# dubhater/vapoursynth-mvtools

Measured on AMD Instinct MI355X. Metric: MDegrain3 cfg3 fps (Super+Analyse+Degrain end-to-end), higher is better.
Workload: dtype u16; 1 GPU; 4K YUV420P16 Degrain3 blksize=16 overlap=8 pel=2; batches_in_flight=2

## Files before the change

vapoursynth-mvtools_amd/csrc/mvx_analyse_spec.h:

```cpp
#pragma once
#include <type_traits>
#include "mvx_analyse_fast.h"

#define SPEC_TB 32
#define SPEC_STRIDE (SPEC_TB * 8 + 8)
#define SPEC_SLOTS_HEX 19
#define SPEC_SLOTS_EXH 29
#define MVX_FAST_NOSTRIP 8
#define MVX_FAST_NOSPEC 4

#ifdef MVX_SPEC_NOPACK
#define MVX_SPEC_PACK 0
#else
#define MVX_SPEC_PACK 1
#endif
#ifndef MVX_SPEC_PLANEORDER
#define MVX_SPEC_PLANEORDER 1
#endif
constexpr int SPEC_SW3 = 12;
#ifdef MVX_SPEC_PROF
#define SPROF_N 20
static __device__ unsigned long long g_specprof[SPROF_N];
#define SPROF(i) do { const long long t1_ = (long long)__builtin_amdgcn_s_memtime(); asm volatile("s_waitcnt lgkmcnt(0)" : : "s"(t1_) : "memory"); sprof[i] += t1_ - sprofT; sprofT = t1_; } while (0)
#else
#define SPROF(i) ((void)0)
#endif
#ifdef MVX_SPEC_PROF
#define SPEC_PROF_DUMP_() do { if (l == 0 && chain == 5 && S.role == 1) for (int i = 0; i < SPROF_N; i++) g_specprof[i] = (unsigned long long)S.sprof[i]; } while (0)
#else
#define SPEC_PROF_DUMP_() ((void)0)
#endif
#ifdef MVX_SPEC_STATS
static __device__ unsigned long long g_specstat[MVX_MAX_LEVELS][10];
#endif

template <int BPS, int BW, bool UV, int SWIN = 12, bool TEAM = false, bool SIDE = false> struct SpecSearcher : FastSearcher<BPS, BW, UV, 48> {
    typedef FastSearcher<BPS, BW, UV, 48> F;
    typedef FGeo<BPS, BW> G;
    using F::P; using F::J; using F::lds; using F::ldsRow; using F::ldsHist; using F::histBins;
    using F::nBlkX; using F::nBlkY; using F::pel; using F::logPel; using F::pw; using F::ph; using F::hpad; using F::vpad;
    using F::srcY; using F::srcU; using F::srcV; using F::refY; using F::refU; using F::refV; using F::srcUV; using F::refUV;
    using F::pitchY; using F::pitchC; using F::pstrideY; using F::pstrideC; using F::shadowY; using F::vectors;
    using F::chroma; using F::searchType; using F::nSearchParam; using F::penaltyNew; using F::penaltyZero; using F::pglobal; using F::badrange; using F::badcount; using F::fieldShift;
    using F::badSAD; using F::LSAD; using F::gmvx; using F::gmvy;
    using F::x0; using F::y0; using F::blkIdx; using F::nDxMin; using F::nDyMin; using F::nDxMax; using F::nDyMax;
    using F::predX; using F::predY; using F::pX; using F::pY; using F::nLambda; using F::bestX; using F::bestY; using F::bestSad;
    int ldsTab;
    int role, nw;
    lds_u8 *shRow;
    LDS_AS int *ctl;
    __device__ __forceinline__ int team_advance(int g, int c0, int lo, int hiE, bool fwd, int stepX, int hps) const {
        auto clampAt = [&](int v, int li) { const int xb = stepX * (c0 + li); return min(max(v, -((xb + hps) << logPel)), ((pw - xb - hpad - BW - hpad + hps) << logPel) - 1); };
        if (clampAt(g, lo) == g && clampAt(g, hiE - 1) == g) return g;
        for (int i = 0; i < hiE - lo; i++) g = clampAt(g, fwd ? lo + i : hiE - 1 - i);
        return g;
    }
    __device__ __forceinline__ void team_wait_ge(int need) const {
#ifdef MVX_TEAM_WATCHDOG
        unsigned spins = 0;
#endif
        while (uni(__hip_atomic_load(ctl, __ATOMIC_ACQUIRE, __HIP_MEMORY_SCOPE_WORKGROUP)) < need) {
            __builtin_amdgcn_s_sleep(2);
#ifdef MVX_TEAM_WATCHDOG
            if (++spins > (1u << 26)) __builtin_trap();
#endif
        }
    }
    __device__ __forceinline__ void team_acquire(int myG, int &px, int &py, int &ps) {
        team_wait_ge(myG);
        px = uni(__hip_atomic_load(ctl + 1, __ATOMIC_RELAXED, __HIP_MEMORY_SCOPE_WORKGROUP));
        py = uni(__hip_atomic_load(ctl + 2, __ATOMIC_RELAXED, __HIP_MEMORY_SCOPE_WORKGROUP));
        ps = uni(__hip_atomic_load(ctl + 3, __ATOMIC_RELAXED, __HIP_MEMORY_SCOPE_WORKGROUP));
        badcount = uni(__hip_atomic_load(ctl + 4, __ATOMIC_RELAXED, __HIP_MEMORY_SCOPE_WORKGROUP));
    }
    __device__ __forceinline__ void team_release(int done, int px, int py, int ps) const {
        if (lane_id() == 0) {
            __hip_atomic_store(ctl + 1, px, __ATOMIC_RELAXED, __HIP_MEMORY_SCOPE_WORKGROUP);
            __hip_atomic_store(ctl + 2, py, __ATOMIC_RELAXED, __HIP_MEMORY_SCOPE_WORKGROUP);
            __hip_atomic_store(ctl + 3, ps, __ATOMIC_RELAXED, __HIP_MEMORY_SCOPE_WORKGROUP);
            __hip_atomic_store(ctl + 4, badcount, __ATOMIC_RELAXED, __HIP_MEMORY_SCOPE_WORKGROUP);
        }
        __builtin_amdgcn_fence(__ATOMIC_RELEASE, "workgroup");
        if (lane_id() == 0) __hip_atomic_store(ctl, done, __ATOMIC_RELEASE, __HIP_MEMORY_SCOPE_WORKGROUP);
    }
#ifdef MVX_SPEC_PROF
    long long sprof[SPROF_N], sprofT;
// ... 38 lines not shown
        oA = luma_off_at(bx0, vx, vy) + (unsigned)rowA * pitchY + (unsigned)xbA;
        oB = 2 * chroma_off_at(bx0, vx, vyc) + (unsigned)rowB * 2 * pitchC + (unsigned)xbB;
    }
    template <int LOGG, int WMAX> __device__ __forceinline__ v4u pass_issue(Pass<LOGG, WMAX> &T, int piece) const {
        typedef PG<LOGG, WMAX> Q;
        v4u v;
        if (piece < Q::NA) { v = F::template ld_ref<G::LCB>(refY + T.curA); T.curA += (unsigned)(Q::GG >> G::LLOGC) * pitchY; asm volatile("" : "+v"(T.curA) : : "memory"); }
        else { v = F::template ld_ref<G::UVCB>(refUV + T.curB); T.curB += (unsigned)(Q::GG >> G::UVLOGC) * 2 * pitchC; asm volatile("" : "+v"(T.curB) : : "memory"); }
        return v;
    }
    template <int LOGG, int WMAX> __device__ __forceinline__ void pass_prime(Pass<LOGG, WMAX> &T, unsigned oA, unsigned oB) const {
        typedef PG<LOGG, WMAX> Q;
        T.curA = oA; T.curB = oB;
#pragma unroll
        for (int k = 0; k < Q::W; k++) T.r[k] = pass_issue(T, k);
    }
    template <int LOGG, int WMAX, bool REFILL = true> __device__ __forceinline__ void pass_run(Pass<LOGG, WMAX> &T, int s, unsigned nA, unsigned nB) const {
        typedef PG<LOGG, WMAX> Q;
        const int rowA = s >> G::LLOGC, xbA = (s & (Q::CA - 1)) * G::LCB, rowB = s >> G::UVLOGC, xbB = (s & (Q::CB - 1)) * G::UVCB;
        const lds_u8 *spA = lds + rowA * G::LROWB + xbA, *spB = lds + G::UOFF + rowB * G::UVROWB + xbB;
        constexpr int lstepA = (Q::GG >> G::LLOGC) * G::LROWB, lstepB = (Q::GG >> G::UVLOGC) * G::UVROWB;
        auto src_piece = [&](int k) { return k < Q::NA ? F::template lds_piece<G::LCB>(spA + k * lstepA) : F::template lds_piece<G::UVCB>(spB + (k - Q::NA) * lstepB); };
        constexpr int D = MVX_SRC_AHEAD < Q::NT ? MVX_SRC_AHEAD : Q::NT;
        v4u a[D];
#pragma unroll
        for (int k = 0; k < D; k++) a[k] = src_piece(k);
        unsigned aL = 0, aC = 0;
#pragma unroll
        for (int k = 0; k < Q::NT; k++) {
            const v4u cur = a[k % D];
            if (k + D < Q::NT) a[k % D] = src_piece(k + D);
            if (k < Q::NA) aL = F::template sad_regs<G::LCB>(cur, T.r[k % Q::W], aL);
            else aC = F::template sad_regs<G::UVCB>(cur, T.r[k % Q::W], aC);
            asm volatile("" : "+v"(aL), "+v"(aC) : : "memory");
            const int kk = k + Q::W;
            if (kk == Q::NT) { T.curA = nA; T.curB = nB; }
            if (REFILL || kk < Q::NT) T.r[k % Q::W] = pass_issue(T, kk % Q::NT);
        }
        T.aL = aL; T.aC = aC;
    }

#ifndef MVX_STRIP32
#define MVX_STRIP32 0
#endif
    static constexpr bool STRIP_OK = (BPS == 2 && (BW == 16 || (MVX_STRIP32 && BW == 32))) || (BPS == 1 && BW == 16);
    static constexpr int COLB = BPS == 2 ? 16 : 8, ROWB = 8 * COLB;
    static constexpr int HC = STRIP_OK ? BW / 16 : 1, SW_BLOCKS = 8 / HC - 1, LPB = 2 * HC, LPC = SW_BLOCKS * LPB;
    static constexpr int pickSW(int nt, int w) { return w <= 1 ? 1 : (w <= nt && nt % w == 0) ? w : pickSW(nt, w - 1); }
    static constexpr int SNA = BW, SNB = UV ? BW / 2 : 0, SNT = SNA + SNB, SW = pickSW(SNT, (BW == 32 && SWIN > 12) ? 12 : SWIN), S_UV = SNA * ROWB, SSTG = SNT / 8;
    static constexpr bool SDMA = STRIP_OK && COLB == 16 && HC == 1 && SW == 24 && SNT == 24;
    static_assert(!SDMA || (SW == SNT && SSTG == 3), "SDMA: strip_run<true> issues exactly SW loads per pass, a strip is three loads per lane");
    static_assert(SW <= 63, "the wait for a strip is s_waitcnt vmcnt(SW)");
    static constexpr bool PACK = SDMA && MVX_SPEC_PACK;
    __device__ __forceinline__ static int hex_ord(int i) {
        if constexpr (MVX_SPEC_PLANEORDER != 0) return (int)(0xDCBA7630985421ull >> (4 * i)) & 15;
        else return i;
    }
    struct StripPass { v4u r[SW]; unsigned curA, curB, aL, aC; };
    __device__ __forceinline__ v4u strip_issue(StripPass &T, int piece) const {
        v4u v;
        if (piece < SNA) { v = F::template ld_ref<COLB>(refY + T.curA); T.curA += pitchY; asm volatile("" : "+v"(T.curA) : : "memory"); }
        else { v = F::template ld_ref<COLB>(refUV + T.curB); T.curB += 2 * pitchC; asm volatile("" : "+v"(T.curB) : : "memory"); }
        return v;
    }
    __device__ __forceinline__ void strip_prime(StripPass &T, unsigned oA, unsigned oB) const {
        T.curA = oA; T.curB = oB;
#pragma unroll
        for (int k = 0; k < SW; k++) T.r[k] = strip_issue(T, k);
    }
    template <bool REFILL> __device__ __forceinline__ void strip_run(StripPass &T, int p, unsigned nA, unsigned nB, int bufOff = 0) const {
        const lds_u8 *sp = lds + bufOff + p * COLB;
        auto src_piece = [&](int k) { return F::template lds_piece<COLB>(sp + (k < SNA ? k * ROWB : S_UV + (k - SNA) * ROWB)); };
        constexpr int D = MVX_SRC_AHEAD;
        v4u a[D];
#pragma unroll
        for (int k = 0; k < D; k++) a[k] = src_piece(k);
        unsigned aL = 0, aC = 0;
#pragma unroll
        for (int k = 0; k < SNT; k++) {
            const v4u cur = a[k % D];
            if (k + D < SNT) a[k % D] = src_piece(k + D);
            if (k < SNA) aL = F::template sad_regs<COLB>(cur, T.r[k % SW], aL);
            else aC = F::template sad_regs<COLB>(cur, T.r[k % SW], aC);
            asm volatile("" : "+v"(aL), "+v"(aC) : : "memory");
            const int kk = k + SW;
            if (kk == SNT) { T.curA = nA; T.curB = nB; }
            if (REFILL || kk < SNT) T.r[k % SW] = strip_issue(T, kk % SNT);
        }
        T.aL = aL; T.aC = aC;
    }
    static constexpr bool STRIP8_OK = UV && BPS == 1 && BW == 8;
    static constexpr int W8_BLOCKS = 15, R8A = 8, R8B = 4, R8T = R8A + R8B;
    static_assert(!SIDE || (STRIP_OK && HC == 1) || STRIP8_OK, "blocks side by side: the 16x16 and the 8-bit 8x8 row passes only");
    static constexpr int WBLK = STRIP_OK ? (SIDE ? 4 : SW_BLOCKS) : STRIP8_OK ? (SIDE ? 8 : W8_BLOCKS) : SPEC_TB;
    static constexpr int GT = SPEC_TB / WBLK * WBLK, FR = 2 * GT;
    static_assert(GT >= 1 && GT <= SPEC_TB && FR <= 64, "a group fits the table, a frame the wave");
    struct Strip8 { v4u r[R8T]; unsigned curA, curB; unsigned aL[4], aC[4]; };
    __device__ __forceinline__ v4u strip8_issue(Strip8 &T, int piece) const {
        v4u v;
        if (piece < R8A) { v = F::template ld_ref<16>(refY + T.curA); T.curA += pitchY; asm volatile("" : "+v"(T.curA) : : "memory"); }
        else { v = F::template ld_ref<16>(refUV + T.curB); T.curB += 2 * pitchC; asm volatile("" : "+v"(T.curB) : : "memory"); }
        return v;
    }
    __device__ __forceinline__ void strip8_prime(Strip8 &T, unsigned oA, unsigned oB) const {
        T.curA = oA; T.curB = oB;
#pragma unroll
// ... 65 lines not shown
        __builtin_amdgcn_s_barrier();

        if (smallestPlane) { searchType = P.nLevels == 1 ? P.searchType : P.searchTypeCoarse; nSearchParam = P.nLevels == 1 ? P.nPelSearch : P.nSearchParam; }
        else { searchType = lvl == 0 ? P.searchType : P.searchTypeCoarse; nSearchParam = lvl == 0 ? P.nPelSearch : P.nSearchParam; }
        searchType = uni(searchType); nSearchParam = uni(nSearchParam);
        fieldShift = uni(lvl == 0 ? J.fieldShift : 0);
        badSAD = uni(P.badSAD); badrange = uni(P.badrange); badcount = 0;
        gmvx = pel * globalX; gmvy = pel * globalY + fieldShift;
        int nLambdaLevel = P.lambda / (pel * pel);
        const int nScale = 1 << lvl;
        if (P.plevel == 1) nLambdaLevel = nLambdaLevel * nScale;
        else if (P.plevel == 2) nLambdaLevel = nLambdaLevel * nScale * nScale;
        nLambdaLevel = uni(nLambdaLevel);
        penaltyZero = uni(P.pzero); pglobal = uni(P.global ? P.pglobal : P.pzero); penaltyNew = uni(P.pnew); LSAD = uni((long long)P.lsad);
        const int stepX = uni(P.blkX - P.ovX), stepY = uni(P.blkY - P.ovY);
        const int hps = hpad >> lvl, vps = vpad >> lvl;
        const bool meander = uni(P.meander) != 0;
        LDS_AS v2u *rowbuf = (LDS_AS v2u *)(TEAM ? shRow : lds + ldsRow);
        lds_u8 *tab = TEAM ? lds + ldsTab : lds + ldsRow + ((nBlkX * 8 + 15) & ~15);
        this->pf_setup();
        SPROF(8);
        auto lambda_of = [&](int predSad) {
            const double scale = (double)LSAD / (double)(LSAD + (long long)(predSad >> 1));
            return (int)(long long)((double)(long long)nLambdaLevel * scale * scale);
        };
        const bool hexLevel = searchType == SearchHex2;
        const bool specLevel = specEnabled && !smallestPlane;
        int rdx = 0, rdy = 0;
        if (hexLevel) {
            const int g = l >> 2;
            if (g < 6) { rdx = tab8(HEX2X >> 8, g & 7); rdy = tab8(HEX2Y >> 8, g & 7); }
            else if (g < 14) { rdx = tab8(PACK8(0, 0, -1, 1, -1, -1, 1, 1), g - 6); rdy = tab8(PACK8(-1, 1, 0, 0, -1, 1, -1, 1), g - 6); }
        } else {
            const int g = l >> 1, k = g < 8 ? g : g - 8;
            if (g < 8) { rdx = tab8(PACK8(0, 0, -1, 1, -1, -1, 1, 1), k); rdy = tab8(PACK8(-1, 1, 0, 0, -1, 1, -1, 1), k); }
            else if (g < 16) { rdx = tab8(PACK8(-1, -1, 0, 0, 1, 1, -2, 2), k); rdy = tab8(PACK8(-2, 2, -2, 2, -2, 2, -1, -1), k); }
            else if (g < 24) { rdx = tab8(PACK8(-2, 2, -2, 2, -2, -2, 2, 2), k - 8); rdy = tab8(PACK8(0, 0, 1, 1, -2, 2, -2, 2), k - 8); }
        }
        unsigned sPat = 0, bPat0 = 0, bPat1 = 0;
        {
            constexpr bool side8 = STRIP8_OK && SIDE;
            constexpr bool side16 = SIDE;
            const int gb = side8 ? l >> 3 : STRIP8_OK ? (l >= 45 ? 3 : l >= 30 ? 2 : l >= 15 ? 1 : 0) : side16 ? min(l >> 3, 3) : min(l / LPC, 3);
            for (int q = 0; q < 8; q++) {
                int dx, dy;
                const int sIdx = STRIP8_OK ? q * 16 + (l >> 2) : (PACK && hexLevel && q >= 1) ? 8 + (8 * (q - 1) + (l >> 3)) % 6 : q * 8 + (l >> 3);
                if (q < 4) { pat_delta(hexLevel, (STRIP_OK && hexLevel) ? hex_ord(min(sIdx, 13)) : sIdx, dx, dy); sPat |= (unsigned)((dx & 15) | ((dy & 15) << 4)) << (8 * q); }
                pat_delta(hexLevel, q * (side8 ? 8 : 4) + gb, dx, dy);
                const unsigned b = (unsigned)((dx & 15) | ((dy & 15) << 4)) << (8 * (q & 3));
                if (q < 4) bPat0 |= b; else bPat1 |= b;
            }
        }
#ifdef MVX_SPEC_STATS
        unsigned long long st0 = 0, st1 = 0, st2 = 0, st3 = 0, st4 = 0, st5 = 0, st6 = 0, st7 = 0, st8 = 0, st9 = 0;
#endif

        int prevX = 0, prevY = 0, prevSad = 0;
        const int syncGroups = syncEvery > 0 ? max(1, (syncEvery + GT / 2) / GT) : 0;
        int syncCount = syncGroups - 1;
        int Gc = 0;
        const int nGrpRow = (nBlkX + GT - 1) / GT;
        for (int blky = 0; blky < nBlkY; blky++) {
            const bool fwd = (blky & 1) == 0 || !meander;
            const int dir = fwd ? 1 : -1;
            y0 = vpad + stepY * blky;
            nDyMax = (ph - y0 - BW - vpad + vps) << logPel;
            nDyMin = -((y0 - vpad + vps) << logPel);
            if constexpr (TEAM) gmvy = this->clipy(gmvy);
            const bool specRow = specLevel && blky > 0;
            const int ngrp = (nBlkX + FR - 1) / FR;
            for (int gi = 0; gi < ngrp; gi++) {
                const int grp = fwd ? gi : ngrp - 1 - gi;
                const int c0 = grp * FR, c = c0 + l;
                const int ncol = min(FR, nBlkX - c0);
                const bool in = l < ncol;
                v4u bOut = {0, 0, 0, 0};
                for (int hi = 0; hi < 2; hi++) {
                    const int h = fwd ? hi : 1 - hi;
                    const int lo = h * GT, hiE = min(lo + GT, ncol);
                    if (lo >= ncol) continue;
                    const int myG = Gc++;
                    bool teamHeld = false;
                    if constexpr (TEAM) {
                        if (uni(myG % nw) != role) {
                            gmvx = team_advance(gmvx, c0, lo, hiE, fwd, stepX, hps);
                            continue;
                        }
                        if (specRow) {
                            const int j = 2 * grp + h;
                            const bool fwdPrev = ((blky - 1) & 1) == 0 || !meander;
                            auto idxPrev = [&](int jj) { return fwdPrev ? jj : nGrpRow - 1 - jj; };
                            int need = (blky - 1) * nGrpRow + idxPrev(j) + 1;
                            if (blky == nBlkY - 1) { const int j2 = j + dir; if (j2 >= 0 && j2 < nGrpRow) need = max(need, (blky - 1) * nGrpRow + idxPrev(j2) + 1); }
                            SPROF(7);
                            team_wait_ge(need);
                            SPROF(16);
                        }
                    }
                    SPROF(7);
                    if (syncGroups && ++syncCount == syncGroups) { __builtin_amdgcn_s_barrier(); syncCount = 0; }
                    SPROF(0);
                    const bool act = l >= lo && l < hiE;
                    unsigned long long okmask = 0, flagmask = 0;
                    int rX = 0, rY = 0, rSad = 0;
                    int pkU = 0, pkAh = 0, pkH = 0, pkG = 0;
                    int lam = 0;
                    bool staged2G = false;
// ... 74 lines not shown
                                    }
                                }
#pragma unroll
                                for (int k = 0; k < 8; k++) {
                                    const int vx = wx + tab8(PACK8(0, 0, -1, 1, -1, -1, 1, 1), k), vy = wy + tab8(PACK8(-1, 1, 0, 0, -1, 1, -1, 1), k);
                                    const v2u t = tt[6 + k];
                                    const int cc = cnew(vx, vy, t);
                                    if (vok(vx, vy) && cc < best) { best = cc; bx = vx; by = vy; bs = tot(t); }
                                }
                            } else {
#pragma unroll 1
                                for (int k0 = 0; k0 < 24; k0 += 8) {
                                    v2u tt[8];
#pragma unroll
                                    for (int k = 0; k < 8; k++) tt[k] = rd(k0 + k);
#pragma unroll
                                    for (int k = 0; k < 8; k++) {
                                        int dx, dy;
                                        if (k0 == 0) { dx = tab8(PACK8(0, 0, -1, 1, -1, -1, 1, 1), k); dy = tab8(PACK8(-1, 1, 0, 0, -1, 1, -1, 1), k); }
                                        else if (k0 == 8) { dx = tab8(PACK8(-1, -1, 0, 0, 1, 1, -2, 2), k); dy = tab8(PACK8(-2, 2, -2, 2, -2, 2, -1, -1), k); }
                                        else { dx = tab8(PACK8(-2, 2, -2, 2, -2, -2, 2, 2), k); dy = tab8(PACK8(0, 0, 1, 1, -2, 2, -2, 2), k); }
                                        const int vx = wx + dx, vy = wy + dy;
                                        const v2u t = tt[k];
                                        const int cc = cnew(vx, vy, t);
                                        if (vok(vx, vy) && cc < best) { best = cc; bx = vx; by = vy; bs = tot(t); }
                                    }
                                }
                            }
                            return won;
                        };
                        bool staged2 = false;
                        int pBest = 0, pX_ = 0, pY_ = fieldShift, pSad = 0;

                        const int nb = hiE - lo;
                        const bool lumaStrips = STRIP_OK && !UV && !chroma && stripEnabled && stepX == (SIDE ? BW : BW / 2);
                        const bool streamed = (chroma && (hexLevel ? STREAM_HEX : STREAM_EXH)) || lumaStrips;
                        if (streamed) {
                            const int pkZ = pk(0, fieldShift);
                            const int slotUp = hexLevel ? 14 : 24, slotZ = hexLevel ? 16 : 26;
                            unsigned long long pbMask = __ballot(act), p3Mask = 0;

                            SPROF(1);
                            if constexpr (STRIP_OK) {
                                constexpr bool side = SIDE;
                                if (stripEnabled && stepX == (side ? BW : BW / 2) && (UV ? chroma != 0 : chroma == 0)) {
                                    constexpr int TC = side ? 2 : HC, SWB = side ? 4 : SW_BLOCKS, LPCr = SWB * LPB;
                                    static_assert(SWB == WBLK, "the group length is counted in these windows");
                                    const int nw = (nb + SWB - 1) / SWB;
                                    const int npat = hexLevel ? 14 : 24;
                                    pbMask = 0;
                                    staged2 = true;
                                    unsigned stripW = 0;
                                    unsigned packS = 0;
                                    int pkW = 0;
                                    int lq = l;
                                    asm volatile("" : "+v"(lq));
                                    int gS, pS, gB, rB, mB, hB;
                                    bool tail, idleB;
                                    auto roles = [&]() {
                                        lq = l;
                                        asm volatile("" : "+v"(lq));
                                        gS = lq >> 3; pS = lq & 7;
                                        gB = side ? min(lq >> 3, 3) : min(lq / LPC, 3);
                                        rB = side ? (lq & 7) : lq >= 4 * LPC ? (lq - 4 * LPC) % LPC : lq - LPC * gB; mB = rB / LPB; hB = rB % LPB;
                                        tail = lq >= 56; idleB = lq >= 4 * LPCr;
                                    };
                                    roles();
                                    constexpr int SBUF = SNT * ROWB;
                                    auto widx = [&](int i) { return fwd ? i : nw - 1 - i; };
                                    auto w_cand = [&](int st, int w, int q, int rj, int &slot, int &colW, bool &stripLane, int &srcOff, unsigned &oA, unsigned &oB) {
                                        const int f = lo + SWB * w, L = min(SWB, hiE - f);
                                        const int bxf = hpad + stepX * (c0 + f);
                                        const int bufW = SDMA ? (widx(w) & 1) * SBUF : 0;
                                        const bool stripWin = st == 2 && ((stripW >> w) & 1);
                                        const int meB = min(mB, L - 1), colB = f + meB;
                                        int bU = 0, bAh = 0, bG = 0, bH = 0, bW = 0;
                                        if (st == 1) {
                                            bU = __builtin_amdgcn_ds_bpermute(colB << 2, pkU); bAh = __builtin_amdgcn_ds_bpermute(colB << 2, pkAh);
                                            bG = __builtin_amdgcn_ds_bpermute(colB << 2, pkG); bH = __builtin_amdgcn_ds_bpermute(colB << 2, pkH);
                                        } else if (!stripWin) bW = __builtin_amdgcn_ds_bpermute(colB << 2, pkW);
                                        if (stripWin || (st == 1 && tail)) {
                                            const int p = st == 1 ? pS : pS, g = gS;
                                            int vx, vy, vyc;
                                            int fV = f, LV = L, bxV = bxf, bufV = bufW;
                                            if (st == 1) { vx = 0; vy = fieldShift; vyc = 0; slot = slotZ; }
                                            else {
                                                int sW = __builtin_amdgcn_readlane(pkW, f);
                                                int idx = q * 8 + g, sh = 8 * q;
                                                if constexpr (PACK) {
                                                    if (rj >= 0) {
                                                        const int w2 = widx(widx(w) + 1), f2 = lo + SWB * w2, L2 = min(SWB, hiE - f2);
                                                        const int sW2 = __builtin_amdgcn_readlane(pkW, f2);
                                                        const bool hi = g >= 6 - 2 * rj;
                                                        fV = hi ? f2 : f; LV = hi ? L2 : L; bxV = hpad + stepX * (c0 + fV); sW = hi ? sW2 : sW; bufV = hi ? SBUF - bufW : bufW;
                                                        idx = 8 + 2 * rj + g - (hi ? 6 : 0); sh = 8 * (1 + rj);
                                                    }
                                                }
                                                const int dd = (int)(sPat >> sh), dx = (dd << 28) >> 28, dy = (dd << 24) >> 28;
                                                vx = upx(sW) + dx; vy = upy(sW) + dy; vyc = vy;
                                                slot = idx < npat ? (hexLevel ? hex_ord(idx) : idx) : -1;
                                            }
                                            const int pe = min(p, TC * (LV - 1) + 2 * HC - 1) * COLB;
                                            if ((p % TC != 0) | (p / TC >= LV)) slot = -1;
                                            colW = fV + p / TC; stripLane = true; srcOff = bufV + p * COLB;
                                            oA = luma_off_at(bxV, vx, vy) + (unsigned)pe;
                                            oB = 2 * chroma_off_at(bxV, vx, vyc) + (unsigned)pe;
                                        } else {
                                            const int me = meB, col = colB;
                                            int base, dx = 0, dy = 0;
                                            if (st == 1) {
                                                base = gB == 0 ? bU : gB == 1 ? bAh : gB == 2 ? bG : bH;
                                                slot = gB == 0 ? slotUp : gB == 1 ? slotUp + 1 : slotZ + gB - 1;
                                            } else {
                                                base = bW;
                                                const int ci = q * 4 + gB;
                                                const int dd = (int)((q < 4 ? bPat0 : bPat1) >> (8 * (q & 3)));
                                                dx = (dd << 28) >> 28; dy = (dd << 24) >> 28;
                                                slot = ci < npat ? ci : -1;
                                            }
                                            const int bx0 = hpad + stepX * (c0 + col);
                                            const int xMax = (pw - bx0 - BW - hpad + hps) << logPel, xMin = -((bx0 - hpad + hps) << logPel);
                                            const int cxv = upx(base), cyv = upy(base), tx = cxv + dx, ty = cyv + dy;
                                            const bool ok = (tx >= xMin) & (ty >= nDyMin) & (tx < xMax) & (ty < nDyMax);
                                            const int vx = ok ? tx : cxv, vy = ok ? ty : cyv;
                                            if ((hB != 0) | (mB >= L) | idleB) slot = -1;
                                            colW = f + me; stripLane = false; srcOff = bufW + (TC * me + hB) * COLB;
                                            oA = luma_off_at(bx0, vx, vy) + (unsigned)(hB * COLB);
                                            oB = 2 * chroma_off_at(bx0, vx, vy) + (unsigned)(hB * COLB);
                                        }
                                    };
                                    A4x32 stg[SDMA ? 1 : SSTG];
                                    auto stage_issue = [&](int w, int buf) {
                                        const int f = lo + SWB * w, L = min(SWB, hiE - f), bx0 = hpad + stepX * (c0 + f), pe = min(pS, TC * (L - 1) + 2 * HC - 1) * COLB;
                                        if constexpr (SDMA) asm volatile("s_waitcnt lgkmcnt(0)" : : : "memory");
#pragma unroll
                                        for (int k = 0; k < SSTG; k++) {
                                            const int row = gS + 8 * k;
                                            gl_u8 *g = 8 * k < SNA ? srcY + (unsigned)(y0 + row) * pitchY + (unsigned)bx0 * BPS + (unsigned)pe
                                                                   : srcUV + (unsigned)((y0 >> 1) + row - SNA) * 2 * pitchC + (unsigned)(bx0 >> 1) * 2 * BPS + (unsigned)pe;
                                            if constexpr (SDMA) {
                                                const unsigned m0v = (unsigned)(unsigned long long)(lds + buf * SBUF + 8 * k * ROWB);
                                                asm volatile("s_mov_b32 m0, %1\n\tglobal_load_lds_dwordx4 %0, off" : : "v"(g), "s"(m0v) : "memory", "m0");
                                            } else stg[k] = ld_chunk_g(g, COLB);
                                        }
                                    };
                                    auto stage_store = [&]() {
                                        if constexpr (SDMA) asm volatile("s_waitcnt vmcnt(%0)" : : "n"(SW) : "memory");
                                        else {
#pragma unroll
                                            for (int k = 0; k < SSTG; k++) st_chunk_l(lds + (gS + 8 * k) * ROWB + pS * COLB, stg[k], COLB);
                                        }
                                    };
                                    auto npass = [&](int st, int w) { return st == 1 ? 1 : ((stripW >> w) & 1) ? (npat + 7) / 8 : (npat + 3) / 4; };
                                    auto run_stage = [&](int st, int wFrom, int wTo) {
                                        int wi = wFrom, w = widx(wFrom), q = 0, rj = -1, ci = -1;
                                        if constexpr (PACK) ci = (st == 2 && ((packS >> wi) & 1)) ? 0 : -1;
                                        StripPass T;
                                        int slot, colW, srcOff; bool stripLane; unsigned oA, oB;
                                        roles();
                                        w_cand(st, w, q, rj, slot, colW, stripLane, srcOff, oA, oB);
                                        if constexpr (SDMA) { stage_issue(w, wi & 1); strip_prime(T, oA, oB); }
                                        else { strip_prime(T, oA, oB); stage_issue(w, 0); }
                                        for (;;) {
                                            roles();
                                            int wn = w, qn = q + 1, win = wi, rjn = -1, cin = ci;
                                            bool nextWin;
                                            if (PACK && ci >= 0) {
                                                if (rj < 0 && ci < 3) { rjn = ci; nextWin = false; }
                                                else { cin = ci < 3 ? ci + 1 : -1; nextWin = true; }
                                            } else nextWin = qn >= npass(st, w);
                                            if (nextWin) {
                                                qn = 0; win = wi + 1; wn = widx(win);
                                                if constexpr (PACK) { if (st == 2 && cin < 0 && win < wTo && ((packS >> win) & 1)) cin = 0; }
                                            }
                                            const bool more = win < wTo;
                                            int slotN = -1, colN = 0, srcN = 0; bool stripN = false; unsigned nA = 0, nB = 0;
                                            SPROF(2);
                                            if (more) w_cand(st, wn, qn, rjn, slotN, colN, stripN, srcN, nA, nB);
                                            SPROF(11);
                                            if (q == 0 || (PACK && rj >= 0)) {
                                                __builtin_amdgcn_wave_barrier();
                                                stage_store();
                                                if (q == 0 && wi + 1 < wTo) stage_issue(widx(wi + 1), (wi + 1) & 1);
                                                __builtin_amdgcn_wave_barrier();
                                            }
                                            SPROF(12);
                                            if (more) strip_run<true>(T, 0, nA, nB, srcOff); else strip_run<false>(T, 0, 0, 0, srcOff);
                                            SPROF(13);
                                            unsigned sL = T.aL + (unsigned)__builtin_amdgcn_update_dpp(0, (int)T.aL, 0x101, 0xf, 0xf, true), sC = T.aC + (unsigned)__builtin_amdgcn_update_dpp(0, (int)T.aC, 0x101, 0xf, 0xf, true);
                                            unsigned hL = T.aL + (unsigned)__builtin_amdgcn_update_dpp(0, (int)T.aL, 0xB1, 0xf, 0xf, true), hC = T.aC + (unsigned)__builtin_amdgcn_update_dpp(0, (int)T.aC, 0xB1, 0xf, 0xf, true);
                                            if (HC == 2) {
                                                sL += (unsigned)__builtin_amdgcn_update_dpp(0, (int)sL, 0x102, 0xf, 0xf, true); sC += (unsigned)__builtin_amdgcn_update_dpp(0, (int)sC, 0x102, 0xf, 0xf, true);
                                                hL += (unsigned)__builtin_amdgcn_update_dpp(0, (int)hL, 0x4E, 0xf, 0xf, true); hC += (unsigned)__builtin_amdgcn_update_dpp(0, (int)hC, 0x4E, 0xf, 0xf, true);
                                            }
                                            if (slot >= 0) *(LDS_AS v2u *)(tab + slot * SPEC_STRIDE + (colW & (SPEC_TB - 1)) * 8) = v2u{stripLane ? sL : hL, stripLane ? sC : hC};
                                            SPROF(14);
#ifdef MVX_SPEC_PROF
                                            sprof[15] += 1;
#endif
#ifdef MVX_SPEC_STATS
                                            if (st == 2) st8 += 1;
#endif
                                            if (!more) break;
                                            w = wn; wi = win; q = qn; rj = rjn; ci = cin; slot = slotN; colW = colN; stripLane = stripN; srcOff = srcN;
                                        }
                                        __builtin_amdgcn_wave_barrier();
                                    };
                                    run_stage(1, 0, nw);
                                    a2_pred(pBest, pX_, pY_, pSad);
                                    pkW = pk(pX_, pY_);
                                    {
                                        const bool ok2 = (pX_ - 2 >= dxMin) & (pX_ + 2 <= dxMax1) & (pY_ - 2 >= nDyMin) & (pY_ + 2 < nDyMax);
                                        for (int w = 0; w < nw; w++) {
                                            const int f = lo + SWB * w, e = min(f + SWB, hiE);
                                            const bool inw = (l >= f) & (l < e);
                                            const int w0 = __builtin_amdgcn_readlane(pkW, f);
                                            if (e - f >= 2 && __ballot(inw & ((pkW != w0) | !ok2)) == 0) stripW |= 1u << w;
#ifdef MVX_SPEC_STATS
                                            if ((stripW >> w) & 1) st4 += 1;
                                            else { st5 += 1; st6 += __builtin_popcountll(__ballot(inw & (pkW != w0))); if (__ballot(inw & (pkW != w0)) == 0) st7 += 1; }
#endif
                                        }
                                        if constexpr (PACK) {
                                            if (hexLevel) {
                                                for (int i = 0; i + 4 <= nw;) {
                                                    bool all4 = true;
                                                    for (int k = 0; k < 4; k++) all4 = all4 && ((stripW >> widx(i + k)) & 1);
                                                    if (all4) { packS |= 1u << i; i += 4; } else i++;
                                                }
                                            }
#if defined(MVX_SPEC_STATS)
                                            st9 += __builtin_popcount(packS);
#endif
                                        }
                                    }
                                    run_stage(2, 0, nw);
                                }
                            }

                            if constexpr (STRIP8_OK) {
                                auto rows8 = [&](auto DS2) {
                                    constexpr bool ds2 = decltype(DS2)::value;
                                    const int wmax = ds2 ? 8 : W8_BLOCKS;
                                    static_assert((ds2 ? 8 : W8_BLOCKS) == WBLK, "the group length is counted in these windows");
                                    const int nw = (nb + wmax - 1) / wmax, WL = (nb + nw - 1) / nw;
                                    const int npat = hexLevel ? 14 : 24;
                                    pbMask = 0;
                                    staged2 = true;
                                    unsigned stripW = 0;
                                    int pkW = 0;
                                    int lq, gS, qS, gB, mB;
                                    bool tail;
                                    auto roles = [&]() {
                                        lq = l;
                                        asm volatile("" : "+v"(lq));
                                        gS = lq >> 2; qS = lq & 3;
                                        if (ds2) { gB = lq >> 3; mB = lq & 7; }
                                        else { gB = min(lq / W8_BLOCKS, 3); mB = lq >= 60 ? lq - 60 : lq - W8_BLOCKS * gB; }
                                        tail = lq >= 60;
                                    };
                                    roles();
                                    auto w_cand = [&](int st, int w, int q, int &slot, int &colW, int &nwr, int &srcA, int &srcB, int &shA, int &shB, unsigned &oA, unsigned &oB) {
                                        const int f = lo + WL * w, L = min(WL, hiE - f);
                                        const int bxf = hpad + stepX * (c0 + f);
                                        const bool stripWin = st == 2 && ((stripW >> w) & 1);
                                        const int meB = min(mB, L - 1), colB = f + meB;
                                        int bU = 0, bAh = 0, bG = 0, bH = 0, bW = 0;
                                        if (st == 1) {
                                            bU = __builtin_amdgcn_ds_bpermute(colB << 2, pkU); bAh = __builtin_amdgcn_ds_bpermute(colB << 2, pkAh);
                                            bG = __builtin_amdgcn_ds_bpermute(colB << 2, pkG); bH = __builtin_amdgcn_ds_bpermute(colB << 2, pkH);
// ... 411 lines not shown
                            nLambda = 0;
                            if (blky > 0) nLambda = uni(lambda_of(predSad));
                            if (specRow) { const int g = __builtin_amdgcn_readlane(pkG, li); gmvx = upx(g); gmvy = upy(g); }
                            __builtin_amdgcn_wave_barrier();
                            this->pf_store(sb);
                            __builtin_amdgcn_wave_barrier();
                            this->search_block();
                            __builtin_amdgcn_wave_barrier();
                            { const bool mine = l == li; bOut[0] = mine ? (unsigned)bestX : bOut[0]; bOut[1] = mine ? (unsigned)bestY : bOut[1]; bOut[2] = mine ? (unsigned)bestSad : bOut[2]; }
                            prevX = bestX; prevY = bestY; prevSad = bestSad;
#ifdef MVX_SPEC_STATS
                            if (specRow) { st0 += 1; st1 += 1; st2 += !((flagmask >> li) & 1); }
#endif
                            SPROF(6);
#ifdef MVX_SPEC_PROF
                            sprof[10] += 1;
#endif
                            const int nx = pos + dir;
                            if (specRow && nx != end) {
                                const int xb = stepX * (c0 + nx);
                                const int u = __builtin_amdgcn_readlane(pkU, nx);
                                const int lx = min(max(bestX, -((xb + hps) << logPel)), ((pw - xb - hpad - BW - hpad + hps) << logPel) - 1);
                                const bool hyp = lx == upx(u) && this->clipy(bestY) == upy(u);
                                const unsigned long long bit = 1ull << nx;
                                okmask = (hyp && (flagmask & bit)) ? (okmask | bit) : (okmask & ~bit);
                            }
                            pos += dir;
                        }
                    }
                    if (specRow) gmvx = gEndX;
                    if constexpr (TEAM) {
                        if (act) {
                            typedef unsigned a4v __attribute__((ext_vector_type(4), aligned(4)));
                            const a4v t = {bOut[0], bOut[1], bOut[2], 0u};
                            *(GL_AS a4v *)&vectors[blky * nBlkX + c] = t;
                            rowbuf[c] = v2u{(unsigned)pk((int)bOut[0], (int)bOut[1]), bOut[2]};
                        }
                        team_release(myG + 1, prevX, prevY, prevSad);
                    }
                    SPROF(5);
#ifdef MVX_SPEC_PROF
                    sprof[9] += 1;
#endif
                }
                if (!TEAM && in) {
                    typedef unsigned a4v __attribute__((ext_vector_type(4), aligned(4)));
                    const a4v t = {bOut[0], bOut[1], bOut[2], 0u};
                    *(GL_AS a4v *)&vectors[blky * nBlkX + c] = t;
                    rowbuf[c] = v2u{(unsigned)pk((int)bOut[0], (int)bOut[1]), bOut[2]};
                }
            }
        }
#ifdef MVX_SPEC_STATS
        if (l == 0) { atomicAdd(&g_specstat[lvl][0], st0); atomicAdd(&g_specstat[lvl][1], st1); atomicAdd(&g_specstat[lvl][2], st2); atomicAdd(&g_specstat[lvl][3], st3); atomicAdd(&g_specstat[lvl][4], st4); atomicAdd(&g_specstat[lvl][5], st5); atomicAdd(&g_specstat[lvl][6], st6); atomicAdd(&g_specstat[lvl][7], st7); atomicAdd(&g_specstat[lvl][8], st8); atomicAdd(&g_specstat[lvl][9], st9); }
#endif
        SPROF(7);
        __builtin_amdgcn_fence(__ATOMIC_RELEASE, "workgroup");
        __builtin_amdgcn_fence(__ATOMIC_ACQUIRE, "workgroup");
        __builtin_amdgcn_s_barrier();
    }
};

template <int BPS, int BW, int WPE, int MAXCPW, bool UV, bool TEAM = false, bool SIDE = false>
__global__ __launch_bounds__(64 * MAXCPW, WPE) void analyse_spec_kernel(const AParams *Pp, const AJob *jobs, int njobs, int ldsChain, int syncEvery, int ldsRow, int ldsHist, int histBins, int ldsTab, int flags) {
    extern __shared__ __attribute__((aligned(16))) unsigned char smem[];
    const AParams &P = *Pp;
    const int cpw = TEAM ? 1 : (int)(blockDim.x >> 6);
    int wg = (int)blockIdx.x;
    if (flags & MVX_FAST_XCD_REMAP) {
        const int n = (int)gridDim.x, x = wg & 7, slot = wg >> 3;
        wg = x * (n >> 3) + min(x, n & 7) + slot;
    }
    const int wave = uni((int)(threadIdx.x >> 6));
    const int chain = uni(TEAM ? wg : wg * cpw + wave);
    if (chain >= njobs) return;
    const AJob &J = jobs[chain];
    if (!J.blob) return;
    const int l = lane_id();
    int *hdr = (int *)J.blob;
    if (TEAM && wave != 0 && !J.valid) return;
    if (!J.valid) {
        if (l == 0) { hdr[0] = P.blobSize; hdr[1] = 0; }
        for (int lvl = P.nLevels - 1; lvl >= 0; lvl--) {
            const ALevel &L = P.lv[lvl];
            unsigned char *rec = J.blob + L.blobOff;
            const int nBlk = L.nBlkX * L.nBlkY;
            if (l == 0) *(int *)rec = 4 + nBlk * 16;
            GVec *v = (GVec *)(rec + 4);
            for (int i = l; i < nBlk; i += WAVE) { GVec d; d.x = 0; d.y = 0; d.sad = P.verybigSAD; v[i] = d; }
        }
        return;
    }
    if (l == 0 && (!TEAM || wave == 0)) { hdr[0] = P.blobSize; hdr[1] = 1; }
    SpecSearcher<BPS, BW, UV, (WPE <= 2 ? 24 : SPEC_SW3), TEAM, SIDE> S(P, J);
    S.lds = (lds_u8 *)smem + (TEAM ? ldsRow : 0) + wave * ldsChain;
    S.ldsRow = ldsRow; S.ldsHist = ldsHist; S.histBins = histBins; S.ldsTab = ldsTab;
    S.role = wave; S.nw = uni((int)(blockDim.x >> 6)); S.ctl = (LDS_AS int *)((lds_u8 *)smem); S.shRow = (lds_u8 *)smem + 64;
#ifdef MVX_SPEC_PROF
    for (int i = 0; i < SPROF_N; i++) S.sprof[i] = 0;
    S.sprofT = (long long)__builtin_amdgcn_s_memtime();
#endif
    int gx = 0, gy = 0;
    GL_AS const GVec *coarse = nullptr;
    int cbx = 0, cby = 0, clp = 0;
    for (int lvl = P.nLevels - 1; lvl >= 0; lvl--) {
        if (coarse && P.global) S.estimate_global(coarse, cbx * cby, 8192 * P.lv[lvl + 1].pel, &gx, &gy);
        S.search_level_spec(lvl, gx, gy, coarse, cbx, cby, clp, (cpw > 1 && !TEAM) ? syncEvery : 0, !(flags & MVX_FAST_NOSPEC), !(flags & MVX_FAST_NOSTRIP));
        coarse = S.vectors; cbx = P.lv[lvl].nBlkX; cby = P.lv[lvl].nBlkY; clp = P.lv[lvl].logPel;
    }
    SPEC_PROF_DUMP_();
}
#ifdef MVX_SPEC_PROF
#define SPEC_PROF_DUMP() do { if (l == 0 && chain == 5) for (int i = 0; i < SPROF_N; i++) g_specprof[i] = (unsigned long long)S.sprof[i]; } while (0)
#else
#define SPEC_PROF_DUMP() ((void)0)
#endif
#if defined(MVX_SPEC_PROF) && defined(MVX_PROF_EXPORT)
extern "C" __attribute__((visibility("default"))) int mvx_debug_specprof(unsigned long long *out) {
    return hipMemcpyFromSymbol(out, HIP_SYMBOL(g_specprof), sizeof(unsigned long long) * SPROF_N) == hipSuccess ? 0 : -1;
}
#endif
#if defined(MVX_SPEC_STATS) && defined(MVX_PROF_EXPORT)
extern "C" __attribute__((visibility("default"))) int mvx_debug_specstats(unsigned long long *out, int reset) {
    if (hipMemcpyFromSymbol(out, HIP_SYMBOL(g_specstat), sizeof(unsigned long long) * MVX_MAX_LEVELS * 10) != hipSuccess) return -1;
    if (reset) { static unsigned long long z[MVX_MAX_LEVELS * 10]; if (hipMemcpyToSymbol(HIP_SYMBOL(g_specstat), z, sizeof(z)) != hipSuccess) return -1; }
    return 0;
}
#endif

struct ASpecLaunch { ALaunch L; int ldsTab; int team; int side; };
template <int BPS, int BW, int WPE, int MAXCPW, bool UV, bool SIDE = false> static int launch_analyse_spec_uv(const ASpecLaunch &S) {
    const ALaunch &L = S.L;
    const int perChain = (L.ldsNeed + 255) & ~255;
    const int cpw = L.cpw < MAXCPW ? L.cpw : MAXCPW;
    const int lds = perChain * cpw;
    if (lds > 64 * 1024)
        HIP_CHECK(hipFuncSetAttribute((const void *)analyse_spec_kernel<BPS, BW, WPE, MAXCPW, UV, false, SIDE>, hipFuncAttributeMaxDynamicSharedMemorySize, lds));
    hipLaunchKernelGGL((analyse_spec_kernel<BPS, BW, WPE, MAXCPW, UV, false, SIDE>), dim3((L.njobs + cpw - 1) / cpw), dim3(64 * cpw), lds, L.st, L.dP, L.dJobs,
                       L.njobs, perChain, L.syncEvery, L.ldsRow, L.ldsHist, L.histBins, S.ldsTab, L.flags);
    return MVX_OK;
}
template <int BPS, int BW, int WPE, int MAXCPW, bool SIDE = false> static int launch_analyse_spec(const ASpecLaunch &S) {
    if (S.L.flags & MVX_FAST_UV) return launch_analyse_spec_uv<BPS, BW, WPE, MAXCPW, true, SIDE>(S);
    return launch_analyse_spec_uv<BPS, BW, WPE, MAXCPW, false, SIDE>(S);
}
template <int BPS, int BW, int WPE, int MAXCPW, bool UV, bool SIDE = false> static int launch_analyse_spec_team_uv(const ASpecLaunch &S) {
    const ALaunch &L = S.L;
    const int nw = S.team < MAXCPW ? S.team : MAXCPW;
    const int perWave = (L.ldsNeed + 255) & ~255;
    const int lds = L.ldsRow + perWave * nw;
    if (lds > 64 * 1024)
        HIP_CHECK(hipFuncSetAttribute((const void *)analyse_spec_kernel<BPS, BW, WPE, MAXCPW, UV, true, SIDE>, hipFuncAttributeMaxDynamicSharedMemorySize, lds));
    hipLaunchKernelGGL((analyse_spec_kernel<BPS, BW, WPE, MAXCPW, UV, true, SIDE>), dim3(L.njobs), dim3(64 * nw), lds, L.st, L.dP, L.dJobs,
                       L.njobs, perWave, 0, L.ldsRow, L.ldsHist, L.histBins, S.ldsTab, L.flags);
    return MVX_OK;
}
template <int BPS, int BW, int WPE, int MAXCPW, bool SIDE = false> static int launch_analyse_spec_team(const ASpecLaunch &S) {
    if (S.L.flags & MVX_FAST_UV) return launch_analyse_spec_team_uv<BPS, BW, WPE, MAXCPW, true, SIDE>(S);
    return launch_analyse_spec_team_uv<BPS, BW, WPE, MAXCPW, false, SIDE>(S);
}
```

Baseline: 1010 fps.

## Add run-form speculative search for windows with few distinct predictor runs

Adds a 'run' mode to the speculative strip search. Windows whose predictors form two or three contiguous runs of equal vectors, and which are not near the search limits, are now processed as strip-like passes that share loads across the columns of each run. Before, such windows fell back to the per-column path, which needs more passes. The change also alters the DPP reduction pattern when RUN is compiled in and adds stat counters. It brings more lane-mapping logic and readlanes, and any mismatch between the chosen DPP pattern and the lane layout could affect correctness.

```diff
diff --git a/vapoursynth-mvtools_amd/csrc/mvx_analyse_spec.h b/vapoursynth-mvtools_amd/csrc/mvx_analyse_spec.h
--- a/vapoursynth-mvtools_amd/csrc/mvx_analyse_spec.h
+++ b/vapoursynth-mvtools_amd/csrc/mvx_analyse_spec.h
@@ -13,6 +13,14 @@
 #define MVX_SPEC_PACK 0
 #else
 #define MVX_SPEC_PACK 1
+#endif
+#ifdef MVX_SPEC_NORUN
+#define MVX_SPEC_RUN 0
+#else
+#define MVX_SPEC_RUN 1
+#endif
+#ifndef MVX_SPEC_RUNMAX
+#define MVX_SPEC_RUNMAX 3
 #endif
 #ifndef MVX_SPEC_PLANEORDER
 #define MVX_SPEC_PLANEORDER 1
@@ -31,7 +39,8 @@
 #define SPEC_PROF_DUMP_() ((void)0)
 #endif
 #ifdef MVX_SPEC_STATS
-static __device__ unsigned long long g_specstat[MVX_MAX_LEVELS][10];
+#define SPEC_NSTAT 17
+static __device__ unsigned long long g_specstat[MVX_MAX_LEVELS][SPEC_NSTAT];
 #endif
 
 template <int BPS, int BW, bool UV, int SWIN = 12, bool TEAM = false, bool SIDE = false> struct SpecSearcher : FastSearcher<BPS, BW, UV, 48> {
@@ -176,6 +185,8 @@
     static_assert(!SDMA || (SW == SNT && SSTG == 3), "SDMA: strip_run<true> issues exactly SW loads per pass, a strip is three loads per lane");
     static_assert(SW <= 63, "the wait for a strip is s_waitcnt vmcnt(SW)");
     static constexpr bool PACK = SDMA && MVX_SPEC_PACK;
+    static constexpr bool RUN = STRIP_OK && !SIDE && HC == 1 && MVX_SPEC_RUN;
+    static_assert(!RUN || SPEC_TB / SW_BLOCKS <= 4, "run form keeps one byte per window of a group");
     __device__ __forceinline__ static int hex_ord(int i) {
         if constexpr (MVX_SPEC_PLANEORDER != 0) return (int)(0xDCBA7630985421ull >> (4 * i)) & 15;
         else return i;
@@ -347,7 +358,7 @@
             }
         }
 #ifdef MVX_SPEC_STATS
-        unsigned long long st0 = 0, st1 = 0, st2 = 0, st3 = 0, st4 = 0, st5 = 0, st6 = 0, st7 = 0, st8 = 0, st9 = 0;
+        unsigned long long st0 = 0, st1 = 0, st2 = 0, st3 = 0, st4 = 0, st5 = 0, st6 = 0, st7 = 0, st8 = 0, st9 = 0, stR[7] = {0, 0, 0, 0, 0, 0, 0};
 #endif
 
         int prevX = 0, prevY = 0, prevSad = 0;
@@ -528,6 +539,7 @@
                                     staged2 = true;
                                     unsigned stripW = 0;
                                     unsigned packS = 0;
+                                    unsigned runW = 0;
                                     int pkW = 0;
                                     int lq = l;
                                     asm volatile("" : "+v"(lq));
@@ -549,11 +561,31 @@
                                         const int bxf = hpad + stepX * (c0 + f);
                                         const int bufW = SDMA ? (widx(w) & 1) * SBUF : 0;
                                         const bool stripWin = st == 2 && ((stripW >> w) & 1);
+                                        const int rb = (RUN && st == 2) ? (int)((runW >> (8 * w)) & 63) : 0;
                                         const int meB = min(mB, L - 1), colB = f + meB;
                                         int bU = 0, bAh = 0, bG = 0, bH = 0, bW = 0;
                                         if (st == 1) {
                                             bU = __builtin_amdgcn_ds_bpermute(colB << 2, pkU); bAh = __builtin_amdgcn_ds_bpermute(colB << 2, pkAh);
                                             bG = __builtin_amdgcn_ds_bpermute(colB << 2, pkG); bH = __builtin_amdgcn_ds_bpermute(colB << 2, pkH);
+                                        } else if (RUN && rb != 0) {
+                                            const int c1 = rb & 7, c2 = rb >> 3;
+                                            const bool r3 = c2 != 0;
+                                            const int g = r3 ? lq / 10 : lq / 9, pos = lq - g * (r3 ? 10 : 9), NC = r3 ? 6 : 7;
+                                            const int idx = q * NC + g, ic = min(idx, npat - 1);
+                                            const int pl = ((ic & 3) * LPC) << 2;
+                                            const unsigned b0 = (unsigned)__builtin_amdgcn_ds_bpermute(pl, (int)bPat0), b1 = (unsigned)__builtin_amdgcn_ds_bpermute(pl, (int)bPat1);
+                                            const int dd = (int)(((ic & 16) ? b1 : b0) >> (8 * ((ic >> 2) & 3))), dx = (dd << 28) >> 28, dy = (dd << 24) >> 28;
+                                            const int r = (pos > c1 ? 1 : 0) + ((r3 & (pos > c2 + 1)) ? 1 : 0);
+                                            const int col = pos - r, colc = min(col, L);
+                                            const int eB = r == 0 ? c1 : (r == 1 && r3) ? c2 : L;
+                                            const int s0 = __builtin_amdgcn_readlane(pkW, f), s1 = __builtin_amdgcn_readlane(pkW, f + c1), s2 = __builtin_amdgcn_readlane(pkW, f + c2);
+                                            const int sW = r == 0 ? s0 : r == 1 ? s1 : s2;
+                                            const int vx = upx(sW) + dx, vy = upy(sW) + dy;
+                                            slot = ((g < NC) & (idx < npat) & (col < eB)) ? idx : -1;
+                                            colW = f + colc; stripLane = true; srcOff = bufW + colc * COLB;
+                                            oA = luma_off_at(bxf, vx, vy) + (unsigned)(colc * COLB);
+                                            oB = 2 * chroma_off_at(bxf, vx, vy) + (unsigned)(colc * COLB);
+                                            return;
                                         } else if (!stripWin) bW = __builtin_amdgcn_ds_bpermute(colB << 2, pkW);
                                         if (stripWin || (st == 1 && tail)) {
                                             const int p = st == 1 ? pS : pS, g = gS;
@@ -627,7 +659,10 @@
                                             for (int k = 0; k < SSTG; k++) st_chunk_l(lds + (gS + 8 * k) * ROWB + pS * COLB, stg[k], COLB);
                                         }
                                     };
-                                    auto npass = [&](int st, int w) { return st == 1 ? 1 : ((stripW >> w) & 1) ? (npat + 7) / 8 : (npat + 3) / 4; };
+                                    auto npass = [&](int st, int w) {
+                                        if (RUN && st == 2 && ((runW >> (8 * w)) & 63)) return (hexLevel && ((runW >> (8 * w)) & 56)) ? 3 : hexLevel ? 2 : 4;
+                                        return st == 1 ? 1 : ((stripW >> w) & 1) ? (npat + 7) / 8 : (npat + 3) / 4;
+                                    };
                                     auto run_stage = [&](int st, int wFrom, int wTo) {
                                         int wi = wFrom, w = widx(wFrom), q = 0, rj = -1, ci = -1;
                                         if constexpr (PACK) ci = (st == 2 && ((packS >> wi) & 1)) ? 0 : -1;
@@ -663,7 +698,8 @@
                                             SPROF(12);
                                             if (more) strip_run<true>(T, 0, nA, nB, srcOff); else strip_run<false>(T, 0, 0, 0, srcOff);
                                             SPROF(13);
-                                            unsigned sL = T.aL + (unsigned)__builtin_amdgcn_update_dpp(0, (int)T.aL, 0x101, 0xf, 0xf, true), sC = T.aC + (unsigned)__builtin_amdgcn_update_dpp(0, (int)T.aC, 0x101, 0xf, 0xf, true);
+                                            constexpr int NEXT = RUN ? 0x130 : 0x101;
+                                            unsigned sL = T.aL + (unsigned)__builtin_amdgcn_update_dpp(0, (int)T.aL, NEXT, 0xf, 0xf, true), sC = T.aC + (unsigned)__builtin_amdgcn_update_dpp(0, (int)T.aC, NEXT, 0xf, 0xf, true);
                                             unsigned hL = T.aL + (unsigned)__builtin_amdgcn_update_dpp(0, (int)T.aL, 0xB1, 0xf, 0xf, true), hC = T.aC + (unsigned)__builtin_amdgcn_update_dpp(0, (int)T.aC, 0xB1, 0xf, 0xf, true);
                                             if (HC == 2) {
                                                 sL += (unsigned)__builtin_amdgcn_update_dpp(0, (int)sL, 0x102, 0xf, 0xf, true); sC += (unsigned)__builtin_amdgcn_update_dpp(0, (int)sC, 0x102, 0xf, 0xf, true);
@@ -676,6 +712,7 @@
 #endif
 #ifdef MVX_SPEC_STATS
                                             if (st == 2) st8 += 1;
+                                            if (RUN && st == 2 && ((runW >> (8 * w)) & 63)) stR[5] += 1;
 #endif
                                             if (!more) break;
                                             w = wn; wi = win; q = qn; rj = rjn; ci = cin; slot = slotN; colW = colN; stripLane = stripN; srcOff = srcN;
@@ -687,11 +724,27 @@
                                     pkW = pk(pX_, pY_);
                                     {
                                         const bool ok2 = (pX_ - 2 >= dxMin) & (pX_ + 2 <= dxMax1) & (pY_ - 2 >= nDyMin) & (pY_ + 2 < nDyMax);
+                                        const int pkWl = __builtin_amdgcn_ds_bpermute((l - 1) << 2, pkW);
                                         for (int w = 0; w < nw; w++) {
                                             const int f = lo + SWB * w, e = min(f + SWB, hiE);
                                             const bool inw = (l >= f) & (l < e);
                                             const int w0 = __builtin_amdgcn_readlane(pkW, f);
                                             if (e - f >= 2 && __ballot(inw & ((pkW != w0) | !ok2)) == 0) stripW |= 1u << w;
+                                            if constexpr (RUN) {
+                                                const unsigned cuts = (unsigned)(__ballot(inw & (l > f) & (pkW != pkWl)) >> f);
+                                                const int R = 1 + __builtin_popcount(cuts);
+                                                const bool lim = __ballot(inw & !ok2) != 0;
+                                                if (!lim && R >= 2 && R <= MVX_SPEC_RUNMAX) {
+                                                    const unsigned rest = cuts & (cuts - 1);
+                                                    runW |= (unsigned)(__builtin_ctz(cuts) | (rest ? __builtin_ctz(rest) << 3 : 0)) << (8 * w);
+                                                }
+#ifdef MVX_SPEC_STATS
+                                                if (!((stripW >> w) & 1)) {
+                                                    stR[lim ? 4 : min(R, 4) - 1] += 1;
+                                                    if ((runW >> (8 * w)) & 63) stR[6] += (npat + 3) / 4 - (hexLevel ? R : 4);
+                                                }
+#endif
+                                            }
 #ifdef MVX_SPEC_STATS
                                             if ((stripW >> w) & 1) st4 += 1;
                                             else { st5 += 1; st6 += __builtin_popcountll(__ballot(inw & (pkW != w0))); if (__ballot(inw & (pkW != w0)) == 0) st7 += 1; }
@@ -1209,7 +1262,7 @@
             }
         }
 #ifdef MVX_SPEC_STATS
-        if (l == 0) { atomicAdd(&g_specstat[lvl][0], st0); atomicAdd(&g_specstat[lvl][1], st1); atomicAdd(&g_specstat[lvl][2], st2); atomicAdd(&g_specstat[lvl][3], st3); atomicAdd(&g_specstat[lvl][4], st4); atomicAdd(&g_specstat[lvl][5], st5); atomicAdd(&g_specstat[lvl][6], st6); atomicAdd(&g_specstat[lvl][7], st7); atomicAdd(&g_specstat[lvl][8], st8); atomicAdd(&g_specstat[lvl][9], st9); }
+        if (l == 0) { atomicAdd(&g_specstat[lvl][0], st0); atomicAdd(&g_specstat[lvl][1], st1); atomicAdd(&g_specstat[lvl][2], st2); atomicAdd(&g_specstat[lvl][3], st3); atomicAdd(&g_specstat[lvl][4], st4); atomicAdd(&g_specstat[lvl][5], st5); atomicAdd(&g_specstat[lvl][6], st6); atomicAdd(&g_specstat[lvl][7], st7); atomicAdd(&g_specstat[lvl][8], st8); atomicAdd(&g_specstat[lvl][9], st9); for (int i = 0; i < 7; i++) atomicAdd(&g_specstat[lvl][10 + i], stR[i]); }
 #endif
         SPROF(7);
         __builtin_amdgcn_fence(__ATOMIC_RELEASE, "workgroup");
@@ -1279,8 +1332,8 @@
 #endif
 #if defined(MVX_SPEC_STATS) && defined(MVX_PROF_EXPORT)
 extern "C" __attribute__((visibility("default"))) int mvx_debug_specstats(unsigned long long *out, int reset) {
-    if (hipMemcpyFromSymbol(out, HIP_SYMBOL(g_specstat), sizeof(unsigned long long) * MVX_MAX_LEVELS * 10) != hipSuccess) return -1;
-    if (reset) { static unsigned long long z[MVX_MAX_LEVELS * 10]; if (hipMemcpyToSymbol(HIP_SYMBOL(g_specstat), z, sizeof(z)) != hipSuccess) return -1; }
+    if (hipMemcpyFromSymbol(out, HIP_SYMBOL(g_specstat), sizeof(unsigned long long) * MVX_MAX_LEVELS * SPEC_NSTAT) != hipSuccess) return -1;
+    if (reset) { static unsigned long long z[MVX_MAX_LEVELS * SPEC_NSTAT]; if (hipMemcpyToSymbol(HIP_SYMBOL(g_specstat), z, sizeof(z)) != hipSuccess) return -1; }
     return 0;
 }
 #endif
```

New measurement: 1038 fps (median of 6 runs). 2.8% higher.
